# Cobalt-27/CompactFusion

Hardware: AMD Instinct MI355X
Metric: residual_compressed_activation_exchange_throughput (higher is better)
Workload: dtype f16

## Files before the change

compactfusion_amd/csrc/cfx_absmean.hip:

```cpp
#include <hip/hip_runtime.h>
#include <hip/hip_ext.h>
#include <stdint.h>
#include <stdio.h>
#include <stdlib.h>
#include <string.h>
#include <algorithm>
#include "cfx.h"
#include "cfx_internal.h"
#include "cfx_device.h"
#include "cfx_host.h"

#define CFX_I_FLAG_LR_FACTORS_ONLY 0x100
#define CFX_I_FLAG_LR_ABS 0x200
extern "C" CFX_HIDDEN size_t cfx_i_lr_workspace_bytes_any(int N, int C, int rank, int batch);
extern "C" CFX_HIDDEN void cfx_i_lr_factor_offsets(int N, int C, int rank, size_t* offU16, size_t* offV16, size_t* per);

template <bool EMIT_BITS, int US, bool WT = false, int NW = WAVES, bool PUB = false, bool KEEP = false, bool TAG = false, class E = ElemF16>
__device__ __forceinline__ void absmean_stats_body(const cfx_comp_item& it, int N, int C, int R, int CB, int bx, int by,
                                                   u64* rowpart, u64 (*sm)[TILE_C], Probe probe = Probe(),
                                                   h16x8* xk = nullptr, h16x8* bk = nullptr, TagArena ta = TagArena()) {
#define SSTAMP(k) probe.at(k)
    const TileCoord t = tile_coord_at(bx, by, N, C, R);
    const int cb = bx;
    u64* colpart = rowpart + (size_t)N * CB;
// ... 259 lines not shown
            const int r = t.r0 + t.w + j * WAVES;
            if (r >= t.r1) continue;
            h16 u[8];
#pragma unroll
            for (int k = 0; k < 8; ++k) u[k] = (k0 + k < K) ? U[(size_t)r * K + k0 + k] : (h16)0;
#pragma unroll
            for (int e = 0; e < 8; ++e)
#pragma unroll
                for (int k = 0; k < 8; ++k) acc[j][e] += (float)(h16)(u[k] * v[e][k]);
        }
    }
#pragma unroll
    for (int j = 0; j < RPT; ++j) {
        const int r = t.r0 + t.w + j * WAVES;
        if (r >= t.r1) continue;
        h16x8 bv = (h16x8)(h16)0, xv = (h16x8)(h16)0;
        if (base) bv = ld8(base + (size_t)r * C + t.c);
        unsigned byte;
        if (QUANT) {
            xv = ld8(x + (size_t)r * C + t.c);
            const h16x8 d = xv - bv;
            byte = 0;
#pragma unroll
            for (int i = 0; i < 8; ++i) byte |= (d[i] >= (h16)0 ? 1u : 0u) << i;
            pk[(size_t)r * C8 + (t.c >> 3)] = (unsigned char)byte;
        } else byte = pk[(size_t)r * C8 + (t.c >> 3)];
        if (!upd) continue;
        h16x8 o;
#pragma unroll
        for (int e = 0; e < 8; ++e) {
            const h16 sc = (h16)acc[j][e];
            const h16 recv = ((byte >> e) & 1u) ? sc : -sc;
            o[e] = base ? (h16)(bv[e] + recv) : recv;
        }
        if (QUANT && !ef) o = xv;
        st8(out + (size_t)r * C + t.c, o);
    }
}

#ifndef WATCH_SLEEP
#define WATCH_SLEEP 4
#endif
#ifndef INT2_FLAG_SLEEP
#define INT2_FLAG_SLEEP 2
#endif
__device__ __forceinline__ void scales_watch(const TagArena& ta, int N, int C, int c0, int r0, long long timeout) {
    const int tid = threadIdx.x;
    if (tid < 2) {
        const u64* w = tid ? ta.tU + min(r0, N - 1) : ta.tV + min(c0 + ((r0 >> 1) & (TILE_C - 1)), C - 1);
        SpinClock clk;
        while (!tag_is(ld_wt(w), ta.tagbits)) {
            __builtin_amdgcn_s_sleep(WATCH_SLEEP);
            if (clk.expired(timeout)) break;
        }
    }
    lds_barrier();
}
template <int ROWS, bool WATCH = true>
__device__ __forceinline__ bool scales_from_tagged(const TagArena& ta, int N, int C, int c0, int r0, u16* s16, long long timeout, unsigned* err) {
    static_assert(ROWS <= TILE_C, "one token word per thread (512 threads = the column block's channels)");
    const int tid = threadIdx.x;
    const u64* pv = ta.tV + min(c0 + tid, C - 1);
    const u64* pu = ta.tU + min(r0 + tid, N - 1);
    SpinClock clk;
    if (WATCH) scales_watch(ta, N, C, c0, r0, timeout);
    for (;;) {
        const u64 v = ld_wt(pv);
        const u64 u = tid < ROWS ? ld_wt(pu) : ta.tagbits;
        const bool ok = tag_is(v, ta.tagbits) && tag_is(u, ta.tagbits);
        s16[tid] = (u16)v;
        if (tid < ROWS) s16[TILE_C + tid] = (u16)u;
        if (!__syncthreads_or(ok ? 0 : 1)) return true;
        __builtin_amdgcn_s_sleep(2);
        if (__syncthreads_or(!ok && clk.expired(timeout) ? 1 : 0)) {
            if (tid == 0) gate_fail(err);
            return false;
        }
    }
}

#ifndef ONEBIT_D_TAGGED
#define ONEBIT_D_TAGGED 0
#endif
template <int NW, int KR, int KL, bool ST, class E = ElemF16>
__device__ __forceinline__ void binary_dequant_gated_body(const cfx_decomp_item& it, int N, int C, int R, int tile_x, int tile_y,
                                                         unsigned* gate, unsigned expect, unsigned* err, long long timeout, u32x4* lds,
                                                         Probe probe = Probe(), bool remote = false, bool tagged = false, TagArena ta = TagArena(),
                                                         u16* s16 = nullptr) {
    constexpr int K = KR + KL;
#define GSTAMP(k) do { if (ST && probe.on()) { asm volatile("s_waitcnt vmcnt(0)" ::: "memory"); probe.at(k); } } while (0)
    const TileCoord t = tile_coord_at(tile_x, tile_y, N, C, R);
    if (ST) { probe.at(0); probe.set(7, 4); }
    const unsigned char* pk = (const unsigned char*)it.packet;
    const int C8 = C >> 3;
    const u16* U = (const u16*)(pk + (size_t)N * C8);
    const u16* V = U + N;
    const h16* base = (const h16*)it.base;
    h16* out = (h16*)it.recon;
    const int cc = min(t.c, C - 8);
    h16x8 bv[KR];
    if (base) {
#pragma unroll
        for (int j = 0; j < KR; ++j) bv[j] = ld8nt(base + (size_t)min(t.r0 + t.w + NW * j, t.r1 - 1) * C + cc);
        if constexpr (KL > 0) {
            h16x8 tl[KL > 0 ? KL : 1];
#pragma unroll
            for (int j = 0; j < KL; ++j) tl[j] = ld8nt(base + (size_t)min(t.r0 + t.w + NW * (KR + j), t.r1 - 1) * C + cc);
#pragma unroll
            for (int j = 0; j < KL; ++j) lds[j * (NW * 64) + threadIdx.x] = __builtin_bit_cast(u32x4, tl[j]);
        }
    } else {
#pragma unroll
        for (int j = 0; j < KR; ++j) bv[j] = (h16x8)(h16)0;
    }
    GSTAMP(1);
    h16x8 v8;
    u16 ul;
    unsigned by[K];
    if (tagged) {
        scales_watch(ta, N, C, tile_x * TILE_C, t.r0, timeout);
        if (ST) probe.at(2);
#pragma unroll
        for (int j = 0; j < K; ++j) by[j] = ld_wt(pk + (size_t)min(t.r0 + t.w + NW * j, t.r1 - 1) * C8 + (cc >> 3));
        if (!scales_from_tagged<NW * K, false>(ta, N, C, tile_x * TILE_C, t.r0, s16, timeout, err)) return;
        v8 = __builtin_bit_cast(h16x8, *(const u16x8*)(s16 + 8 * t.lane));
        ul = s16[TILE_C + min(t.w + NW * min(t.lane, K - 1), t.r1 - 1 - t.r0)];
    } else if (!gate_wait<true>(gate, expect, err, timeout)) return;
    else if (remote) {
        if (ST) probe.at(2);
        u16x8 vb;
#pragma unroll
        for (int i = 0; i < 8; ++i) vb[i] = ld_sys(V + cc + i);
        v8 = __builtin_bit_cast(h16x8, vb);
        ul = ld_sys(U + min(t.r0 + t.w + NW * min(t.lane, K - 1), t.r1 - 1));
#pragma unroll
        for (int j = 0; j < K; ++j) by[j] = ld_sys(pk + (size_t)min(t.r0 + t.w + NW * j, t.r1 - 1) * C8 + (cc >> 3));
    } else {
        if (ST) probe.at(2);
        v8 = ld8_wt(V + cc);
        ul = ld_wt(U + min(t.r0 + t.w + NW * min(t.lane, K - 1), t.r1 - 1));
#pragma unroll
        for (int j = 0; j < K; ++j) by[j] = ld_wt(pk + (size_t)min(t.r0 + t.w + NW * j, t.r1 - 1) * C8 + (cc >> 3));
    }
    GSTAMP(3);
#pragma unroll
    for (int j = 0; j < K; ++j) {
        const int rr = t.r0 + t.w + NW * j;
        const h16 uj = hfrom((u16)__builtin_amdgcn_readlane((int)ul, j));
        if (rr < t.r1 && t.act) {
            const h16x8 s = v8 * uj;
            u16x8 sb = __builtin_bit_cast(u16x8, s);
#pragma unroll
            for (int i = 0; i < 8; ++i) sb[i] ^= ((by[j] >> i) & 1u) ? (u16)0 : (u16)0x8000;
            const h16x8 recv = __builtin_bit_cast(h16x8, sb);
            h16x8 bj = (h16x8)(h16)0;
            if (j < KR) bj = bv[j < KR ? j : 0];
            else if (base) bj = __builtin_bit_cast(h16x8, lds[(j - KR) * (NW * 64) + threadIdx.x]);
            st8nt(out + (size_t)rr * C + t.c, el_state<E>(base != nullptr, bj, recv));
        }
    }
    GSTAMP(4);
#undef GSTAMP
}

__device__ __forceinline__ void row_sums2_wt(const u64* rowpart, const unsigned* row32, int N, int CB, int m0, int m1, bool two, u64& s0, u64& s1) {
    s0 = 0; s1 = 0;
    for (int k0 = 0; k0 < CB; k0 += FUSED_RCH) {
        unsigned a[FUSED_RCH], b[FUSED_RCH];
#pragma unroll
        for (int j = 0; j < FUSED_RCH; ++j) a[j] = ld_wt(&row32[(size_t)min(k0 + j, CB - 1) * N + m0]);
        if (two) {
#pragma unroll
            for (int j = 0; j < FUSED_RCH; ++j) b[j] = ld_wt(&row32[(size_t)min(k0 + j, CB - 1) * N + m1]);
        } else {
#pragma unroll
            for (int j = 0; j < FUSED_RCH; ++j) b[j] = 0;
        }
        bool sat = false;
#pragma unroll
        for (int j = 0; j < FUSED_RCH; ++j) {
            s0 += (k0 + j < CB) ? a[j] : 0; s1 += (k0 + j < CB) ? b[j] : 0;
            sat |= (a[j] == PART_SAT) | (b[j] == PART_SAT);
        }
        if (sat) {
            for (int j = 0; j < FUSED_RCH && k0 + j < CB; ++j) {
                if (a[j] == PART_SAT) s0 += ld_wt(&rowpart[(size_t)(k0 + j) * N + m0]) - (u64)PART_SAT;
                if (two && b[j] == PART_SAT) s1 += ld_wt(&rowpart[(size_t)(k0 + j) * N + m1]) - (u64)PART_SAT;
            }
        }
    }
}

// ... 19 lines not shown
    }
    u64 keep0 = 0, keep1 = 0;
    if (last_all) row_sums2_wt(rowpart, row32, N, CB, min(tid, N - 1), min(tid + NT, N - 1), (tid & ~63) + NT < N, keep0, keep1);
    asm volatile("" ::: "memory");
    STAMP(4);
    u64* smem = &sm[1][0];
    float m0 = 0.f, m1 = 0.f;
    if (last_all) {
        const h16 h0 = mean16(keep0, C), h1 = mean16(keep1, C);
        m0 = (float)h0; m1 = (float)h1;
        u64 acc = 0;
        if (tid < N) acc += habs_units(hbits(h0));
        if (tid + NT < N) acc += habs_units(hbits(h1));
        for (int n0 = tid + 2 * NT; n0 - tid < N; n0 += 2 * NT) {
            const int n1 = n0 + NT;
            u64 s0, s1;
            row_sums2_wt(rowpart, row32, N, CB, min(n0, N - 1), min(n1, N - 1), (n1 & ~63) < N, s0, s1);
            if (n0 < N) acc += habs_units(hbits(mean16(s0, C)));
            if (n1 < N) acc += habs_units(hbits(mean16(s1, C)));
        }
        STAMP(13);
        u64 wtot;
        if (N <= 2 * NT) {
            const unsigned lo = wave_sum_u32_dpp((unsigned)(acc & 0xffffffu));
            const unsigned hi = wave_sum_u32_dpp((unsigned)(acc >> 24));
            wtot = ((u64)hi << 24) + lo;
        } else wtot = wave_sum_u64(acc);
        STAMP(14);
        if ((tid & 63) == 0) smem[tid >> 6] = wtot;
    }
    h16 vmean = (h16)0;
    if (last_col) {
        u64 a = 0;
        for (int p0 = 0; p0 < P; p0 += FUSED_CH) {
            if (p0) {
#pragma unroll
                for (int j = 0; j < FUSED_CH; ++j) v[j] = ld_wt(&col32[(size_t)min(p0 + j, P - 1) * C + cc]);
            }
            bool sat = false;
#pragma unroll
            for (int j = 0; j < FUSED_CH; ++j) { a += (p0 + j < P) ? v[j] : 0; sat |= v[j] == PART_SAT; }
            if (sat) {
                for (int j = 0; j < FUSED_CH && p0 + j < P; ++j)
                    if (v[j] == PART_SAT) a += ld_wt(&colpart[(size_t)(p0 + j) * C + cc]) - (u64)PART_SAT;
            }
        }
        vmean = mean16(a, N);
    }
    STAMP(5);
    if (last_all) {
        lds_barrier();
        STAMP(15);
        u64 tot = 0;
#pragma unroll
        for (int w = 0; w < NT / 64; ++w) tot += smem[w];
        const h16 mu = mean16(tot, N);
        const float den = eps_mode ? (float)(h16)((float)mu + 1e-6f) : (float)mu;
#define PUT16(ptr, val) do { const h16 _v = (val); if (GATED) st_wt((u16*)(ptr), hbits(_v)); else *(ptr) = _v; } while (0)
        if (tid < N) PUT16(&U[tid], (h16)(m0 / den));
        if (tid + NT < N) PUT16(&U[tid + NT], (h16)(m1 / den));
        for (int n0 = tid + 2 * NT; n0 - tid < N; n0 += 2 * NT) {
            const int n1 = n0 + NT;
            u64 s0, s1;
            row_sums2_wt(rowpart, row32, N, CB, min(n0, N - 1), min(n1, N - 1), (n1 & ~63) < N, s0, s1);
            if (n0 < N) PUT16(&U[n0], (h16)((float)mean16(s0, C) / den));
            if (n1 < N) PUT16(&U[n1], (h16)((float)mean16(s1, C) / den));
        }
        if (tid == 0) st_wt(tick + TICK_ALL, 0u);
    }
    if (last_col) {
        if (c < C) PUT16(&V[c], vmean);
        if (tid == 0) st_wt(tick + 1 + bx, 0u);
    }
#undef PUT16
    if (GATED) {
        asm volatile("s_waitcnt vmcnt(0)" ::: "memory");
        lds_barrier();
        if (tid == 0) gate_arrive_few(gate, (last_all ? 1u : 0u) + (last_col ? 1u : 0u));
    }
    STAMP(6);
#undef STAMP
}

__device__ __forceinline__ void absmean_tagged_jobs(const cfx_comp_item& it, int N, int C, int CB, int P, int bx, u64* rowpart, const TagArena& ta,
                                                    int per_byte, int eps_mode, u64 (*sm)[TILE_C], bool do_col, bool do_row, Probe probe,
                                                    unsigned* gate, unsigned* err, long long timeout) {
    constexpr int NT = FUSED_NT;
#define STAMP(k) probe.at(k)
    lds_barrier();
    const int tid = threadIdx.x;
    const u64* colpart = rowpart + (size_t)N * CB;
    h16* U = (h16*)((char*)it.packet + (size_t)N * (C / per_byte));
    h16* V = U + N;
    SpinClock clk;
    bool failed = false;
#define PUT16(ptr, val) st_wt((u16*)(ptr), hbits(val))
    if (do_col) {
        const int c = bx * TILE_C + tid, cc = min(c, C - 1);
        u64 a = 0;
        for (int p0 = 0; p0 < P && !failed; p0 += FUSED_CH) {
            u64 v[FUSED_CH];
            for (;;) {
#pragma unroll
                for (int j = 0; j < FUSED_CH; ++j) v[j] = ld_wt(&ta.tcol[(size_t)min(p0 + j, P - 1) * C + cc]);
                bool ok = true;
#pragma unroll
                for (int j = 0; j < FUSED_CH; ++j) ok = ok && tag_is(v[j], ta.tagbits);
                if (ok) break;
                __builtin_amdgcn_s_sleep(2);
                if (clk.expired(timeout)) { failed = true; break; }
            }
#pragma unroll
            for (int j = 0; j < FUSED_CH; ++j) {
                const u64 w = v[j] & TAG_SAT;
                if (p0 + j < P) a += (w == TAG_SAT && !failed) ? ld_wt(&colpart[(size_t)(p0 + j) * C + cc]) : w;
            }
        }
        STAMP(4);
        failed = __syncthreads_or(failed ? 1 : 0) != 0;
        if (!failed) {
            if (c < C) {
                const h16 vm = mean16(a, N);
                st_wt(&ta.tV[c], ta.tagbits | (u64)hbits(vm));
                PUT16(&V[c], vm);
            }
            asm volatile("s_waitcnt vmcnt(0)" ::: "memory");
            lds_barrier();
            if (tid == 0) gate_arrive_few(gate, 1u);
        }
        STAMP(5);
    }
    if (do_row && !failed) {
        u64* smem = &sm[1][0];
        auto row_sum = [&](int n) {
            const int nc = min(n, N - 1);
            u64 s_ = 0;
            for (int k0 = 0; k0 < CB && !failed; k0 += FUSED_RCH) {
                u64 q[FUSED_RCH];
                for (;;) {
#pragma unroll
                    for (int j = 0; j < FUSED_RCH; ++j) q[j] = ld_wt(&ta.trow[(size_t)min(k0 + j, CB - 1) * N + nc]);
                    bool ok = true;
#pragma unroll
                    for (int j = 0; j < FUSED_RCH; ++j) ok = ok && tag_is(q[j], ta.tagbits);
                    if (ok) break;
                    __builtin_amdgcn_s_sleep(2);
                    if (clk.expired(timeout)) { failed = true; break; }
                }
#pragma unroll
                for (int j = 0; j < FUSED_RCH; ++j) {
                    const u64 w = q[j] & TAG_SAT;
                    if (k0 + j < CB) s_ += (w == TAG_SAT && !failed) ? ld_wt(&rowpart[(size_t)(k0 + j) * N + nc]) : w;
                }
            }
            return s_;
        };
        h16 h0 = (h16)0, h1 = (h16)0;
        u64 acc = 0;
        for (int n0 = tid, i = 0; n0 - tid < N; n0 += NT, ++i) {
            const h16 h = mean16(row_sum(n0), C);
            if (i == 0) h0 = h;
            if (i == 1) h1 = h;
            if (n0 < N) acc += habs_units(hbits(h));
        }
        STAMP(13);
        const u64 wtot = wave_sum_u64(acc);
        if ((tid & 63) == 0) smem[tid >> 6] = wtot;
        failed = __syncthreads_or(failed ? 1 : 0) != 0;
        STAMP(15);
        if (!failed) {
            u64 tot = 0;
#pragma unroll
            for (int w = 0; w < NT / 64; ++w) tot += smem[w];
            const h16 mu = mean16(tot, N);
            const float den = eps_mode ? (float)(h16)((float)mu + 1e-6f) : (float)mu;
            for (int n0 = tid, i = 0; n0 < N; n0 += NT, ++i) {
                const h16 h = i == 0 ? h0 : (i == 1 ? h1 : mean16(row_sum(n0), C));
                const h16 un = (h16)((float)h / den);
                st_wt(&ta.tU[n0], ta.tagbits | (u64)hbits(un));
                PUT16(&U[n0], un);
            }
            asm volatile("s_waitcnt vmcnt(0)" ::: "memory");
            lds_barrier();
            if (tid == 0) gate_arrive_few(gate, 1u);
        }
        STAMP(6);
    }
#undef PUT16
#undef STAMP
    if (failed && tid == 0) gate_fail(err);
}

template <int US, class E = ElemF16>
__device__ __forceinline__ void own_tile_finish(const cfx_comp_item& it, int N, int C, int R, int bx, int by, int flags, const h16x8* xk,
                                                const h16x8* bk, unsigned* gate1, unsigned expect1, unsigned* gate2, unsigned expect2,
                                                unsigned* err, long long timeout, unsigned char* smw, const TagArena& ta, u16* s16) {
    constexpr int NW = FUSED_NW;
    static_assert(US * 8 <= 64, "a wave publishes its US rows of codes with 8 lanes a row");
    const TileCoord t = tile_coord_at(bx, by, N, C, R);
    h16* nb = (h16*)it.new_base;
    const bool upd = (flags & CFX_FLAG_UPDATE_CACHE) && nb;
    const bool ef = !(flags & CFX_FLAG_NO_EF);
    unsigned char* pk = (unsigned char*)it.packet;
    (void)gate1; (void)expect1;
    if (!scales_from_tagged<NW * US>(ta, N, C, bx * TILE_C, t.r0, s16, timeout, err)) return;
    const h16x8 ch8 = __builtin_bit_cast(h16x8, *(const u16x8*)(s16 + 8 * t.lane));
    const u16 ul = s16[TILE_C + min(t.w + NW * min(t.lane, US - 1), t.r1 - 1 - t.r0)];
    const bool has_base = it.base != nullptr;
    u16 codes[US];
#pragma unroll
    for (int j = 0; j < US; ++j) {
        const int rr = t.r0 + t.w + NW * j;
        const h16 tk = hfrom((u16)__builtin_amdgcn_readlane((int)ul, j));
        codes[j] = 0;
        if (rr < t.r1 && t.act) {
            const h16x8 d = el_diff<E>(xk[j], bk[j]);
            const h16x8 thr = ch8 * tk;
            const h16x8 a = habs8(d);
            unsigned code = 0;
#pragma unroll
            for (int i = 0; i < 8; ++i) {
                const unsigned sg = d[i] >= (h16)0 ? 1u : 0u;
                const unsigned m = a[i] > thr[i] ? 1u : 0u;
                code |= ((sg << 1) | m) << (2 * i);
            }
            codes[j] = (u16)code;
            ((u16*)smw)[j * 64 + t.lane] = (u16)code;
        }
    }
    {
        const int j = t.lane >> 3, seg = t.lane & 7;
        const int rr = t.r0 + t.w + NW * j;
        if (t.lane < 8 * US && rr < t.r1 && bx * TILE_C + seg * 64 < C)
            st16_wt(pk + (size_t)rr * (C >> 2) + bx * (TILE_C >> 2) + seg * 16, *(const u32x4*)(smw + j * 128 + seg * 16));
    }
    asm volatile("s_waitcnt vmcnt(0)" ::: "memory");
    lds_barrier();
    if (threadIdx.x == 0) {
        st_wt(&ta.tdone[(size_t)bx * ((N + R - 1) / R) + by], ta.tagbits);
        gate_arrive(gate2, 1u, expect2);
    }
    if (upd) {
#pragma unroll
        for (int j = 0; j < US; ++j) {
            const int rr = t.r0 + t.w + NW * j;
            const h16 tk = hfrom((u16)__builtin_amdgcn_readlane((int)ul, j));
            if (rr < t.r1 && t.act) {
                const h16x8 recv = int2_recv(codes[j], ch8 * tk);
                st8nt(nb + (size_t)rr * C + t.c, ef ? (el_state<E>(has_base, bk[j], recv)) : xk[j]);
            }
        }
    }
}

template <bool EMIT_BITS, int US, bool GATED = false, bool KEEP = false, class E = ElemF16>
__device__ __forceinline__ void absmean_fused_body(const cfx_comp_item& it, int N, int C, int R, int CB, int P, int bx, int by,
                                                   u64* rowpart, unsigned* tick, int per_byte, int eps_mode, u64 (*sm)[TILE_C], int dbg,
                                                   Probe probe, unsigned* gate = nullptr, unsigned gate_expect = 0, int flags = 0,
                                                   unsigned* gate2 = nullptr, unsigned expect2 = 0, unsigned* err = nullptr, long long timeout = 0,
                                                   TagArena ta = TagArena()) {
#define STAMP(k) probe.at(k)
    STAMP(0);
#ifdef CFX_DEV_PROBES
    if (dbg == 3) return;
    if (dbg == 4) {
        const TileCoord t = tile_coord_at(bx, by, N, C, R);
        h16x8 acc = (h16x8)(h16)0;
        for (int r = t.r0 + t.w; r < t.r1; r += FUSED_NW * US) {
            h16x8 xv[US], bv[US];
#pragma unroll
            for (int j = 0; j < US; ++j) {
                const int rr = min(r + FUSED_NW * j, t.r1 - 1);
                xv[j] = ld8nt((const h16*)it.x + (size_t)rr * C + min(t.c, C - 8));
                bv[j] = ld8((const h16*)it.base + (size_t)rr * C + min(t.c, C - 8));
            }
#pragma unroll
            for (int j = 0; j < US; ++j) acc += xv[j] - bv[j];
        }
        if (acc[0] == (h16)12345.0f) ((h16*)it.packet)[threadIdx.x] = acc[1];
        return;
    }
#endif
    h16x8 xk[KEEP ? US : 1], bk[KEEP ? US : 1];
    absmean_stats_body<EMIT_BITS, US, true, FUSED_NW, GATED, KEEP, GATED, E>(it, N, C, R, CB, bx, by, rowpart, sm, probe, xk, bk, ta);
    STAMP(1);
    if constexpr (GATED) {
        const bool v_wg = by == P - 1;
        const bool u_wg = P >= 2 ? (by == P - 2 && bx == CB - 1) : (bx == CB - 1);
        probe.copy(2, 1); probe.copy(3, 1); probe.set(7, (v_wg ? 1 : 0) | (u_wg ? 2 : 0));
        if (v_wg || u_wg) {
            u32x4* park = (u32x4*)&sm[FUSED_NW][0];
            if constexpr (KEEP) {
                park[threadIdx.x] = __builtin_bit_cast(u32x4, xk[US - 1]);
                park[FUSED_NT + threadIdx.x] = __builtin_bit_cast(u32x4, bk[US - 1]);
            }
            absmean_tagged_jobs(it, N, C, CB, P, bx, rowpart, ta, per_byte, eps_mode, sm, v_wg, u_wg, probe, gate, err, timeout);
            if constexpr (KEEP) {
                xk[US - 1] = __builtin_bit_cast(h16x8, park[threadIdx.x]);
                bk[US - 1] = __builtin_bit_cast(h16x8, park[FUSED_NT + threadIdx.x]);
            }
        }
    } else {
    asm volatile("s_waitcnt vmcnt(0)" ::: "memory");
    __syncthreads();
    STAMP(2);
#ifdef CFX_DEV_PROBES
    if (dbg == 1) return;
#endif
    unsigned* flag = (unsigned*)&sm[0][0];
    if (threadIdx.x == 0) flag[0] = __hip_atomic_fetch_add(tick + 1 + bx, 1u, __ATOMIC_RELAXED, __HIP_MEMORY_SCOPE_AGENT);
    if (threadIdx.x == 64) (void)__hip_atomic_fetch_add(tick + TICK_ALL, 1u, __ATOMIC_RELAXED, __HIP_MEMORY_SCOPE_AGENT);
    lds_barrier();
    const bool last_col = flag[0] == (unsigned)(P - 1);
    const bool u_wg = bx == 0 && by == 0;
    STAMP(3);
    probe.set(7, (last_col ? 1 : 0) | (u_wg ? 2 : 0));
#ifdef CFX_DEV_PROBES
    if (dbg == 2) {
        if (last_col && threadIdx.x == 0) st_wt(tick + 1 + bx, 0u);
        if (u_wg && threadIdx.x == 0) {
            while (ld_wt(tick + TICK_ALL) != (unsigned)(CB * P)) __builtin_amdgcn_s_sleep(1);
            st_wt(tick + TICK_ALL, 0u);
        }
        return;
    }
#endif
    if (last_col)
        absmean_last_arriver_jobs<GATED>(it, N, C, CB, P, bx, rowpart, tick, per_byte, eps_mode, sm, true, false, probe, gate, gate_expect);
    if (u_wg) {
        bool failed = false;
        if (threadIdx.x == 0) {
            SpinClock clk;
            while (ld_wt(tick + TICK_ALL) != (unsigned)(CB * P)) {
                __builtin_amdgcn_s_sleep(1);
                if (clk.expired(timeout)) { failed = true; gate_fail(err); break; }
            }
        }
        if (__syncthreads_or(failed ? 1 : 0)) return;
        absmean_last_arriver_jobs<GATED>(it, N, C, CB, P, bx, rowpart, tick, per_byte, eps_mode, sm, false, true, probe, gate, gate_expect);
    }
    }
    if constexpr (KEEP)
        own_tile_finish<US, E>(it, N, C, R, bx, by, flags, xk, bk, gate, gate_expect, gate2, expect2, err, timeout,
                                       (unsigned char*)&sm[__builtin_amdgcn_readfirstlane(threadIdx.x >> 6)][0], ta, (u16*)&sm[FUSED_NW + 4][0]);
#undef STAMP
}

struct FusedArgs {
    int N, C, CB, R, P;
    int n_st;
    int dq_R, dq_rb;
    int per_byte, eps_mode;
    int dbg;
    u64* ws;
    size_t ws_stride;
    unsigned* tick;
    Probe probe;
    int n_g, g_R, g_rb, n_gt;
    unsigned* gate;
    unsigned gate_expect;
    unsigned* gate_err;
    long long timeout;
    u64* tarena; size_t tarena_stride; unsigned tag;
    signed char src[CFX_MAX_BATCH];
    unsigned* xgate;
    unsigned xexpect;
    int remote;
    P2PInline p2p;
};
#ifndef GATE_WPE
#define GATE_WPE 4
#endif
template <bool EMIT_BITS, int US, bool GATED, bool ST, class E>
__global__ __launch_bounds__(FUSED_NT, GATE_WPE) __attribute__((amdgpu_num_vgpr(52))) void k_absmean_compress(BatchC batch, BatchD ride, BatchD gated, FusedArgs a) {
    __shared__ u64 sm[FUSED_NW][TILE_C];
    int b = blockIdx.x;
    if (b < a.n_st) {
        const int per = a.CB * a.P;
        const int z = b / per, rem = b - z * per;
        const int by = rem / a.CB;
        absmean_fused_body<EMIT_BITS, US, GATED, false, E>(batch.it[z], a.N, a.C, a.R, a.CB, a.P, rem - by * a.CB, by, a.ws + (size_t)z * a.ws_stride,
                                                 a.tick + z * TICK_WORDS, a.per_byte, a.eps_mode, sm, a.dbg,
                                                 a.probe.of(b), a.gate, a.gate_expect, 0, nullptr, 0u, a.gate_err, a.timeout,
                                                 tag_arena_of(a.tarena, a.tarena_stride, z, a.N, a.C, a.CB, a.P, a.tag));
        if constexpr (GATED) {
            if (b == 0 && a.p2p.own) p2p_exchange_inline(a.gate, a.gate_expect, 1, a.p2p, a.xgate, a.xexpect, a.gate_err);
        }
        return;
    }
    if constexpr (EMIT_BITS) {
        b -= a.n_st;
        if constexpr (GATED) {
            if (b < a.n_g) {
                const int per = a.CB * a.g_rb;
                for (int t = b; t < a.n_gt; t += a.n_g) {
                    const int item = t / per, rem = t - item * per;
                    const int ty = rem / a.CB;
                    const int sz = a.src[item];
                    const TagArena ta = tag_arena_of(a.tarena, a.tarena_stride, sz >= 0 ? sz : 0, a.N, a.C, a.CB, a.P, a.tag);
                    binary_dequant_gated_body<FUSED_NW, GATE_KR, 0, ST, E>(gated.it[item], a.N, a.C, a.g_R, rem - ty * a.CB, ty, a.xgate ? a.xgate : a.gate,
                                                                a.xgate ? a.xexpect : a.gate_expect, a.gate_err, a.timeout,
                                                                nullptr,
                                                                a.probe.of(blockIdx.x), a.remote != 0 && sz < 0,
                                                                ONEBIT_D_TAGGED && sz >= 0, ta, (u16*)&sm[0][0]);
                }
                return;
            }
            b -= a.n_g;
        }
        const int per = a.CB * a.dq_rb;
        const int item = b / per, rem = b - item * per;
        const int ty = rem / a.CB;
        binary_dequant_body<FUSED_NW, UNROLL, E>(ride.it[item], a.N, a.C, a.dq_R, rem - ty * a.CB, ty);
    }
}

#ifndef PIPE_US
#define PIPE_US 2
#endif
#define PIPE_MAX_DQ CFX_PIPE_MAX_DQ
struct BatchDX { cfx_decomp_item it[PIPE_MAX_DQ]; };
struct PipeArgs {
    int N, C, CB;
    int n_fin, fin_bpi, fin_P;
    int n_st, st_R, st_P;
    int dq_R, dq_rb;
    const u64* ws_fin;
    u64* ws_st;
    size_t ws_stride;
};
template <bool STEADY>
__global__ __launch_bounds__(NTHR) __attribute__((amdgpu_waves_per_eu(8, 8))) void k_binary_pipe(BatchDX dq, BatchC fin, BatchC st, PipeArgs a) {
    __shared__ u64 sm[WAVES][TILE_C];
    int b = blockIdx.x;
    if (b < a.n_fin) {
        const int item = b / a.fin_bpi;
        absmean_finalize_body<NTHR>(fin.it[item], a.N, a.C, a.CB, a.fin_P, 8, 0, a.ws_fin + (size_t)item * a.ws_stride, b - item * a.fin_bpi, &sm[0][0]);
        return;
    }
    b -= a.n_fin;
    if (b < a.n_st) {
        const int per = a.CB * a.st_P;
        const int item = b / per, rem = b - item * per;
        const int ty = rem / a.CB;
        absmean_stats_body<true, PIPE_US>(st.it[item], a.N, a.C, a.st_R, a.CB, rem - ty * a.CB, ty, a.ws_st + (size_t)item * a.ws_stride, sm);
        return;
    }
    b -= a.n_st;
    const int per = a.CB * a.dq_rb;
    const int item = b / per, rem = b - item * per;
    const int ty = rem / a.CB;
    binary_dequant_body<WAVES>(dq.it[item], a.N, a.C, a.dq_R, rem - ty * a.CB, ty);
}


template <class E>
__global__ __launch_bounds__(NTHR) void k_int2_quant(BatchC batch, int N, int C, int R, int flags) {
    const cfx_comp_item it = batch.it[blockIdx.z];
    const TileCoord t = tile_coord(N, C, R);
    const int C4 = C >> 2;
    unsigned char* pk = (unsigned char*)it.packet;
    const h16* TOK = (const h16*)(pk + (size_t)N * C4);
    const h16* CH = TOK + N;
    const h16* x = (const h16*)it.x;
    const h16* base = (const h16*)it.base;
    h16* nb = (h16*)it.new_base;
    const bool upd = (flags & CFX_FLAG_UPDATE_CACHE) && nb;
    const bool ef = !(flags & CFX_FLAG_NO_EF);
    const bool al16 = (((uintptr_t)CH) & 15) == 0;
    h16x8 ch8 = (h16x8)(h16)0;
    if (t.act) ch8 = ld8_tail(CH + t.c, al16);

    for (int r = t.r0 + t.w; r < t.r1; r += WAVES * UNROLL) {
        h16x8 xv[UNROLL], bv[UNROLL];
        h16 tk[UNROLL];
#pragma unroll
        for (int j = 0; j < UNROLL; ++j) {
            const int rr = r + WAVES * j;
            xv[j] = (h16x8)(h16)0; bv[j] = (h16x8)(h16)0; tk[j] = (h16)0;
            if (rr < t.r1 && t.act) {
                xv[j] = ld8nt(x + (size_t)rr * C + t.c);
                if (base) bv[j] = ld8nt(base + (size_t)rr * C + t.c);
                tk[j] = TOK[rr];
            }
        }
#pragma unroll
        for (int j = 0; j < UNROLL; ++j) {
            const int rr = r + WAVES * j;
            if (rr < t.r1 && t.act) {
                const h16x8 d = el_diff<E>(xv[j], bv[j]);
                const h16x8 thr = ch8 * tk[j];
                const h16x8 a = habs8(d);
                unsigned code = 0;
#pragma unroll
                for (int i = 0; i < 8; ++i) {
                    const unsigned s = d[i] >= (h16)0 ? 1u : 0u;
                    const unsigned m = a[i] > thr[i] ? 1u : 0u;
// ... 287 lines not shown
        Int2LayerArgs a;
        memset(&a, 0, sizeof(a));
        a.N = N; a.C = C; a.CB = CB; a.R = R; a.P = P; a.n_st = CB * P * batch;
        a.g_rb = (N + FUSED_NW * (GATE_KR2 + GATE_KL) - 1) / (FUSED_NW * (GATE_KR2 + GATE_KL));
        a.g_R = ((N + a.g_rb - 1) / a.g_rb + FUSED_NW - 1) / FUSED_NW * FUSED_NW;
        a.n_g = CB * a.g_rb * n_gated;
        a.flags = flags; a.ws = ws; a.ws_stride = wstride; a.tick = tick;
        a.gate1 = ctx->gate + (size_t)slot * GATE_STRIDE;
        a.gate2 = a.gate1 + GATE_BLOCK;
        ctx->gate_expect[3 * slot] += (unsigned)batch * (unsigned)(CB + 1);
        ctx->gate_expect[3 * slot + 1] += (unsigned)a.n_st;
        a.expect1 = ctx->gate_expect[3 * slot]; a.expect2 = ctx->gate_expect[3 * slot + 1];
        a.err = ctx->gate_err;
        a.timeout = ctx->gate_timeout;
        a.tarena_stride = tag_arena_words(N, C, CB, P);
        a.tag = abs_arena_for(ctx, slot / TICK_RING, stream, a.tarena_stride * batch * sizeof(u64), &a.tarena);
        if (!a.tag) return fail(ctx, CFX_ERR_LAUNCH, "2-bit layer launch: cannot allocate the partials' arena");
        for (int g_ = 0; g_ < n_gated; ++g_) {
            a.src[g_] = -1;
            for (int i = 0; i < batch; ++i)
                if (gd.it[g_].packet == items[i].packet) a.src[g_] = (signed char)i;
        }
        if (xg) {
            a.xgate = a.gate1 + 2 * GATE_BLOCK;
            a.xexpect = ++ctx->gate_expect[3 * slot + 2];
            a.remote = xg->remote;
            fill_p2p(ctx, xg, a.p2p);
            xg->taken = 1;
            xg->p_gate = a.gate2 + 1 * GATE_LINE;
            xg->p_expect = a.expect2;
            xg->f_gate = a.xgate; xg->f_expect = a.xexpect;
        }
        const dim3 g(a.n_st + a.n_g);
        LAUNCH_EL(bf16, ctx, KID_ABSMEAN_COMPRESS_GATED, s, (k_int2_compress_gated<4, EL>), g, dim3(FUSED_NT), 0, s, b, gd, a);
        return check_launch(ctx, "2-bit layer launch");
    }
    const bool ef_gated = one_launch && codec == CFX_CODEC_BINARY && upd && !(flags & CFX_FLAG_NO_EF) && n_gated + batch <= CFX_MAX_BATCH;
    const bool one_launch_1bit = one_launch && codec == CFX_CODEC_BINARY && (!upd || ef_gated);
    int n_gated_k = n_gated;
    if (ef_gated) {
        for (int i = n_gated - 1; i >= 0; --i) gd.it[i + batch] = gd.it[i];
        for (int i = 0; i < batch; ++i) { gd.it[i].packet = items[i].packet; gd.it[i].base = items[i].base; gd.it[i].recon = items[i].new_base; }
        n_gated_k = n_gated + batch;
    }
    if (fused) {
        FusedArgs a;
        memset(&a, 0, sizeof(a));
        a.N = N; a.C = C; a.CB = CB; a.R = R; a.P = P;
        a.n_st = CB * P * batch;
        a.dq_R = FUSED_NW * UNROLL;
        a.dq_rb = (N + a.dq_R - 1) / a.dq_R;
        a.per_byte = per_byte; a.eps_mode = codec == CFX_CODEC_INT2 ? 1 : 0;
        a.ws = ws; a.ws_stride = wstride; a.tick = tick;
        a.dbg = ctx->dev_probe;
        a.probe = cfx_i_probe(ctx);
        if (one_launch_1bit) {
            a.g_rb = (N + FUSED_NW * GATE_KR - 1) / (FUSED_NW * GATE_KR);
            a.g_R = ((N + a.g_rb - 1) / a.g_rb + FUSED_NW - 1) / FUSED_NW * FUSED_NW;
            a.n_gt = a.n_g = CB * a.g_rb * n_gated_k;
            a.gate = ctx->gate + (size_t)slot * GATE_STRIDE;
            ctx->gate_expect[3 * slot] += (unsigned)batch * (unsigned)(CB + 1);
            a.gate_expect = ctx->gate_expect[3 * slot];
            a.tarena_stride = tag_arena_words(N, C, CB, P);
            a.tag = abs_arena_for(ctx, slot / TICK_RING, stream, a.tarena_stride * batch * sizeof(u64), &a.tarena);
            if (!a.tag) return fail(ctx, CFX_ERR_LAUNCH, "1-bit layer launch: cannot allocate the partials' arena");
            for (int g_ = 0; g_ < n_gated_k; ++g_) {
                a.src[g_] = -1;
                for (int i = 0; i < batch; ++i)
                    if (gd.it[g_].packet == items[i].packet) a.src[g_] = (signed char)i;
            }
            if (xg) {
                a.xgate = a.gate + GATE_BLOCK;
                a.xexpect = ++ctx->gate_expect[3 * slot + 1];
                a.remote = xg->remote;
                fill_p2p(ctx, xg, a.p2p);
                xg->taken = 1;
                xg->p_gate = a.gate; xg->p_expect = a.gate_expect;
                xg->f_gate = a.xgate; xg->f_expect = a.xexpect;
            }
        }
        a.gate_err = ctx->gate_err;
        a.timeout = ctx->gate_timeout;
        const dim3 g(a.n_st + a.n_g + CB * a.dq_rb * n_ride);
#ifdef CFX_DEV_PROBES
        if (one_launch_1bit && ctx->dev_buf && R % 32 == 0) {
            LAUNCH_EL(bf16, ctx, KID_ABSMEAN_COMPRESS_GATED, s, (k_absmean_compress<true, 4, true, true, EL>), g, dim3(FUSED_NT), 0, s, b, rd, gd, a);
        } else
#endif
        if (one_launch_1bit) {
            LAUNCH_EL(bf16, ctx, KID_ABSMEAN_COMPRESS_GATED, s, (k_absmean_compress<true, 4, true, false, EL>), g, dim3(FUSED_NT), 0, s, b, rd, gd, a);
        } else if (codec == CFX_CODEC_BINARY) {
            if (R % 32 == 0) LAUNCH_EL(bf16, ctx, KID_ABSMEAN_COMPRESS_BITS, s, (k_absmean_compress<true, 4, false, false, EL>), g, dim3(FUSED_NT), 0, s, b, rd, gd, a);
            else LAUNCH_EL(bf16, ctx, KID_ABSMEAN_COMPRESS_BITS, s, (k_absmean_compress<true, 2, false, false, EL>), g, dim3(FUSED_NT), 0, s, b, rd, gd, a);
        } else {
            if (R % 32 == 0) LAUNCH_EL(bf16, ctx, KID_ABSMEAN_COMPRESS, s, (k_absmean_compress<false, 4, false, false, EL>), g, dim3(FUSED_NT), 0, s, b, rd, gd, a);
            else LAUNCH_EL(bf16, ctx, KID_ABSMEAN_COMPRESS, s, (k_absmean_compress<false, 2, false, false, EL>), g, dim3(FUSED_NT), 0, s, b, rd, gd, a);
        }
    } else {
        if (codec == CFX_CODEC_BINARY) LAUNCH_EL(bf16, ctx, KID_ABSMEAN_STATS_BITS, s, (k_absmean_stats<true, EL>), grid, dim3(NTHR), 0, s, b, N, C, R, ws, wstride);
        else LAUNCH_EL(bf16, ctx, KID_ABSMEAN_STATS, s, (k_absmean_stats<false, EL>), grid, dim3(NTHR), 0, s, b, N, C, R, ws, wstride);
        LAUNCH(ctx, KID_ABSMEAN_FINALIZE, s, k_absmean_finalize, dim3(1 + (C + 255) / 256, batch), dim3(1024), 0, s, b, N, C, CB, P, per_byte,
                           codec == CFX_CODEC_INT2 ? 1 : 0, (const u64*)ws, wstride);
        if (n_ride) {
            const int Rr = auto_rows(ctx, N, C, n_ride, false);
            LAUNCH_EL(bf16, ctx, KID_BINARY_DEQUANT, s, (k_binary_dequant<UNROLL, EL>), dim3(CB, (N + Rr - 1) / Rr, n_ride), dim3(NTHR), 0, s, rd, N, C, Rr, (unsigned*)nullptr, 0u);
        }
    }
    if (codec == CFX_CODEC_INT2) {
        LAUNCH_EL(bf16, ctx, KID_INT2_QUANT, s, (k_int2_quant<EL>), gridq, dim3(NTHR), 0, s, b, N, C, Rq, flags);
    } else if (upd && !one_launch_1bit) {
        if (flags & CFX_FLAG_NO_EF) {
            for (int i = 0; i < batch; ++i)
                if (items[i].new_base != items[i].x)
                    hipLaunchKernelGGL(k_copy_probe, dim3(2048), dim3(256), 0, s, (uint4*)items[i].new_base, (const uint4*)items[i].x, (size_t)N * C * 2 / 16);
        } else {
            BatchD d;
            memset(&d, 0, sizeof(d));
            for (int i = 0; i < batch; ++i) { d.it[i].packet = items[i].packet; d.it[i].base = items[i].base; d.it[i].recon = items[i].new_base; }
            LAUNCH_EL(bf16, ctx, KID_BINARY_EF, s, (k_binary_dequant<UNROLL, EL>), gridq, dim3(NTHR), 0, s, d, N, C, Rq, (unsigned*)nullptr, 0u);
        }
    }
    if (n_gated && !(one_launch_1bit || (one_launch && codec == CFX_CODEC_INT2))) {
        const int Rg = auto_rows(ctx, N, C, n_gated, false);
        if (codec == CFX_CODEC_BINARY) LAUNCH_EL(bf16, ctx, KID_BINARY_DEQUANT, s, (k_binary_dequant<UNROLL, EL>), dim3(CB, (N + Rg - 1) / Rg, n_gated), dim3(NTHR), 0, s, gd, N, C, Rg, (unsigned*)nullptr, 0u);
        else LAUNCH_EL(bf16, ctx, KID_INT2_DEQUANT, s, (k_int2_dequant<EL>), dim3(CB, (N + Rg - 1) / Rg, n_gated), dim3(NTHR), 0, s, gd, N, C, Rg, (unsigned*)nullptr, 0u);
    }
    return check_launch(ctx, "compress launch");
}

int cfx_i_absmean_decompress(cfx_ctx* ctx, int codec, bool bf16, int N, int C, int batch, const BatchD& b, int R, void* stream, unsigned* pre, unsigned pre_val) {
    hipStream_t s = (hipStream_t)stream;
    const dim3 grid((C + TILE_C - 1) / TILE_C, (N + R - 1) / R, batch);
    if (codec == CFX_CODEC_BINARY) {
        if (stream_cu_count(ctx, stream) < 128) {
            const int R4 = WAVES * 4;
            LAUNCH_EL(bf16, ctx, KID_BINARY_DEQUANT, s, (k_binary_dequant<4, EL>), dim3(grid.x, (N + R4 - 1) / R4, batch), dim3(NTHR), 0, s, b, N, C, R4, pre, pre_val);
        } else LAUNCH_EL(bf16, ctx, KID_BINARY_DEQUANT, s, (k_binary_dequant<UNROLL, EL>), grid, dim3(NTHR), 0, s, b, N, C, R, pre, pre_val);
    } else LAUNCH_EL(bf16, ctx, KID_INT2_DEQUANT, s, (k_int2_dequant<EL>), grid, dim3(NTHR), 0, s, b, N, C, R, pre, pre_val);
    return check_launch(ctx, "decompress launch");
}

extern "C" {

int cfx_int2_quantize(cfx_ctx* ctx, int N, int C, int flags, int batch, const cfx_comp_item* items, void* stream) {
    const bool bf16 = (flags & CFX_FLAG_ELEM_BF16) != 0;
    if (!ctx || !items) return fail(ctx, CFX_ERR_NULL, "int2_quantize: null ctx/items");
    if (batch < 1 || batch > CFX_MAX_BATCH) return fail(ctx, CFX_ERR_BATCH, "int2_quantize: batch out of range");
    if (!shape_ok(CFX_CODEC_INT2, N, C, 0)) return fail(ctx, CFX_ERR_SHAPE, "int2_quantize: bad shape");
    const bool upd = flags & CFX_FLAG_UPDATE_CACHE;
    BatchC b;
    memset(&b, 0, sizeof(b));
    for (int i = 0; i < batch; ++i) {
        if (!items[i].x || !items[i].packet) return fail(ctx, CFX_ERR_NULL, "int2_quantize: null x/packet");
        if (upd && !items[i].new_base) return fail(ctx, CFX_ERR_NULL, "int2_quantize: UPDATE_CACHE needs new_base");
        if (!AL16(items[i].x) || !AL16(items[i].base) || !AL16(items[i].new_base) || !AL16(items[i].packet))
            return fail(ctx, CFX_ERR_ALIGN, "int2_quantize: pointers must be 16-byte aligned");
        b.it[i] = items[i];
    }
    hipStream_t s = (hipStream_t)stream;
    const int Rq = auto_rows(ctx, N, C, batch, true);
    LAUNCH_EL(bf16, ctx, KID_INT2_QUANT, s, (k_int2_quant<EL>), dim3((C + TILE_C - 1) / TILE_C, (N + Rq - 1) / Rq, batch), dim3(NTHR), 0, s, b, N, C, Rq, flags);
    return check_launch(ctx, "int2 quantise launch");
}
}

int cfx_i_launch_pipe(cfx_plan* p, hipStream_t s, int N, int C, const int* comp_op, const int* deq_op,
                       const PipeUnit* dq, const PipeUnit* fin, const PipeUnit* st, int fin_parity, int st_parity,
                       hipEvent_t done_ev) {
    cfx_ctx* ctx = p->ctx;
    BatchDX bd; BatchC bf, bs;
    PipeArgs a;
    memset(&a, 0, sizeof(a));
// ... 118 lines not shown
```

compactfusion_amd/csrc/cfx_device.h:

```cpp
#ifndef CFX_DEVICE_H
#define CFX_DEVICE_H
#include <hip/hip_runtime.h>
#include <stdint.h>
#include "cfx.h"
#include "cfx_internal.h"

typedef _Float16 h16;
typedef h16 h16x8 __attribute__((ext_vector_type(8)));
typedef unsigned short u16;
typedef u16 u16x8 __attribute__((ext_vector_type(8)));
typedef unsigned long long u64;
typedef unsigned u32x4 __attribute__((ext_vector_type(4)));
typedef float f32x2 __attribute__((ext_vector_type(2)));
typedef h16 h16x2 __attribute__((ext_vector_type(2)));
typedef __bf16 bf16x2 __attribute__((ext_vector_type(2)));

#define TILE_C 512
#define WAVES 4
#define NTHR (WAVES * 64)
#define UNROLL 2
#define UNROLL_S 4

struct BatchC { cfx_comp_item it[CFX_MAX_BATCH]; };
struct BatchD { cfx_decomp_item it[CFX_MAX_BATCH]; };
// ... 153 lines not shown
        return __builtin_bit_cast(h16x8, o);
    }
}

template <class E>
__device__ __forceinline__ void el_widen8(h16x8 v, float (&f)[8]) {
    if constexpr (!E::bf16) {
#pragma unroll
        for (int k = 0; k < 8; ++k) f[k] = (float)v[k];
    } else {
        const u32x4 w = __builtin_bit_cast(u32x4, v);
#pragma unroll
        for (int i = 0; i < 4; ++i) {
            const f32x2 p = bf2_f32(w[i]);
            f[2 * i] = p[0];
            f[2 * i + 1] = p[1];
        }
    }
}
template <class E>
__device__ __forceinline__ h16x8 el_round8(const float (&f)[8]) {
    u32x4 o;
#pragma unroll
    for (int i = 0; i < 4; ++i) {
        const f32x2 p = {f[2 * i], f[2 * i + 1]};
        if constexpr (E::bf16) o[i] = f32_bf2(p);
        else o[i] = __builtin_bit_cast(unsigned, __builtin_convertvector(p, h16x2));
    }
    return __builtin_bit_cast(h16x8, o);
}

__device__ __forceinline__ h16x8 int2_recv(u16 code, h16x8 thr) {
    h16x8 r;
#pragma unroll
    for (int i = 0; i < 8; ++i) {
        const unsigned idx = (code >> (2 * i)) & 3u;
        const h16 lvl = (idx & 1u) ? (h16)2.0 * thr[i] : (h16)0.5 * thr[i];
        r[i] = (idx & 2u) ? lvl : -lvl;
    }
    return r;
}

struct TileCoord {
    int lane, w, c, r0, r1;
    bool act;
};
__device__ __forceinline__ TileCoord tile_coord_at(int bx, int by, int N, int C, int R) {
    TileCoord t;
    t.lane = threadIdx.x & 63;
    t.w = __builtin_amdgcn_readfirstlane(threadIdx.x >> 6);
    t.c = bx * TILE_C + t.lane * 8;
    t.act = t.c < C;
    t.r0 = by * R;
    t.r1 = min(N, t.r0 + R);
    return t;
}
__device__ __forceinline__ TileCoord tile_coord(int N, int C, int R) { return tile_coord_at(blockIdx.x, blockIdx.y, N, C, R); }

#define MML_MAX_TILES 2048
#define TICK_WORDS 64
#define TICK_ALL 48
#define TICK_MAX_CB 46
#define TICK_RING 256

#define FUSED_NW 8
#define FUSED_NT (FUSED_NW * 64)
#ifndef FUSED_CH
#define FUSED_CH 18

#endif
#define FUSED_RCH 6

#ifndef GATE_KR
#define GATE_KR 14
#endif
#ifndef GATE_KR2
#define GATE_KR2 17

#endif
#ifndef GATE_KL
#define GATE_KL 6
#endif
#define GATE_LDS_ROWS ((GATE_KL * FUSED_NT * 16 + TILE_C * 8 - 1) / (TILE_C * 8))
#ifndef GATE_LOCAL_SLEEP
#define GATE_LOCAL_SLEEP 1

#endif
#define GATE_LINE 16
#define GATE_BLOCK (25 * GATE_LINE)
#define GATE_STRIDE (3 * GATE_BLOCK)
__device__ __forceinline__ void gate_arrive_few(unsigned* gate, unsigned inc) {
    (void)__hip_atomic_fetch_add(gate, inc, __ATOMIC_RELAXED, __HIP_MEMORY_SCOPE_AGENT);
}
__device__ __forceinline__ void gate_arrive(unsigned* gate, unsigned inc, unsigned expect) {
    const unsigned old = __hip_atomic_fetch_add(gate, inc, __ATOMIC_RELAXED, __HIP_MEMORY_SCOPE_AGENT);
    if (old + inc == expect) {
#pragma unroll
        for (int x = 0; x < 8; ++x) st_wt(gate + (1 + x) * GATE_LINE, expect);
    }
}
__device__ __forceinline__ unsigned ld_l2(const unsigned* p) {
    unsigned v;
    asm volatile("global_load_dword %0, %1, off nt\n\ts_waitcnt vmcnt(0)" : "=&v"(v) : "v"(p) : "memory");
    return v;
}
struct SpinClock {
    long long t0 = 0;
    __device__ __forceinline__ bool expired(long long timeout) {
        const long long now = wall_clock64();
        if (!t0) { t0 = now; return false; }
        return now - t0 > timeout;
    }
};
template <bool FEW = false>
__device__ __forceinline__ bool gate_wait(unsigned* gate, unsigned expect, unsigned* err, long long timeout) {
    bool failed = false;
    if (threadIdx.x == 0) {
        const unsigned xcc = __builtin_amdgcn_s_getreg((3 << 11) | 20) & 7u;
        unsigned* open = FEW ? gate : gate + (1 + xcc) * GATE_LINE;
        unsigned* local = gate + (9 + xcc) * GATE_LINE;
        unsigned* claim = gate + (17 + xcc) * GATE_LINE;
        const bool relay = __hip_atomic_exchange(claim, expect, __ATOMIC_RELAXED, __HIP_MEMORY_SCOPE_AGENT) != expect;
        SpinClock clk;
        unsigned n = 0;
        if (relay) {
            while (ld_wt(open) != expect) {
                __builtin_amdgcn_s_sleep(1);
                if (clk.expired(timeout)) { failed = true; break; }
            }
            if (!failed) *(volatile unsigned*)local = expect;
        } else {
            while (ld_l2(local) != expect) {
                if (GATE_LOCAL_SLEEP) __builtin_amdgcn_s_sleep(GATE_LOCAL_SLEEP);
                ++n;
                if ((n & (FEW ? 255u : 15u)) == 0) {
                    if (ld_wt(open) == expect) break;
                    if (clk.expired(timeout)) { failed = true; break; }
                }
            }
        }
        if (failed) gate_fail(err);
    }
    return __syncthreads_or(failed ? 1 : 0) == 0;
}
__device__ __forceinline__ h16x8 ld8_wt(const u16* p) {
    if ((((uintptr_t)p) & 7) == 0) {
        struct { u64 a, b; } q = {ld_wt((const u64*)p), ld_wt((const u64*)p + 1)};
        return __builtin_bit_cast(h16x8, q);
    }
    u16x8 vb;
#pragma unroll
    for (int i = 0; i < 8; ++i) vb[i] = ld_wt(p + i);
    return __builtin_bit_cast(h16x8, vb);
}

struct P2PInline {
    unsigned* own;
    const unsigned* peer[CFX_P2P_MAX_PEERS];
    int n_peers;
    long long timeout;
};
__device__ __forceinline__ unsigned ld_sys32(const unsigned* p) { return __hip_atomic_load(p, __ATOMIC_RELAXED, __HIP_MEMORY_SCOPE_SYSTEM); }
__device__ __forceinline__ void p2p_exchange_inline(const unsigned* p_gate, unsigned p_expect, int p_count, const P2PInline& p,
                                                    unsigned* f_gate, unsigned f_expect, unsigned* err) {
    if ((threadIdx.x >> 6) != 0) return;
    const int lane = threadIdx.x & 63;
// ... 44 lines not shown
```

Before: 2117.

## Add dense gated compress kernel parking base rows in LDS with staged loads

Adds a k_absmean_compress_dense variant used when the grid fits within a per-CU budget. It keeps fewer base rows in registers (40 VGPRs, higher waves per EU) and parks the remaining rows in shared memory, with each gated block handling exactly one tile instead of looping. It also loads the first rows, waits on them, and then issues the rest. A lean variant of the tagged column wait precomputes a byte offset to cut address arithmetic. The intent is higher occupancy and better latency hiding, at the cost of extra LDS traffic and a forced vmcnt wait.

```diff
diff --git a/compactfusion_amd/csrc/cfx_absmean.hip b/compactfusion_amd/csrc/cfx_absmean.hip
--- a/compactfusion_amd/csrc/cfx_absmean.hip
+++ b/compactfusion_amd/csrc/cfx_absmean.hip
@@ -365,7 +365,7 @@
 #ifndef ONEBIT_D_TAGGED
 #define ONEBIT_D_TAGGED 0
 #endif
-template <int NW, int KR, int KL, bool ST, class E = ElemF16>
+template <int NW, int KR, int KL, bool ST, class E = ElemF16, int STAGE = 0>
 __device__ __forceinline__ void binary_dequant_gated_body(const cfx_decomp_item& it, int N, int C, int R, int tile_x, int tile_y,
                                                          unsigned* gate, unsigned expect, unsigned* err, long long timeout, u32x4* lds,
                                                          Probe probe = Probe(), bool remote = false, bool tagged = false, TagArena ta = TagArena(),
@@ -373,7 +373,7 @@
     constexpr int K = KR + KL;
 #define GSTAMP(k) do { if (ST && probe.on()) { asm volatile("s_waitcnt vmcnt(0)" ::: "memory"); probe.at(k); } } while (0)
     const TileCoord t = tile_coord_at(tile_x, tile_y, N, C, R);
-    if (ST) { probe.at(0); probe.set(7, 4); }
+    if (ST) { probe.at(0); probe.set(7, 4); probe.set(8, (KL << 8) | STAGE); }
     const unsigned char* pk = (const unsigned char*)it.packet;
     const int C8 = C >> 3;
     const u16* U = (const u16*)(pk + (size_t)N * C8);
@@ -383,14 +383,28 @@
     const int cc = min(t.c, C - 8);
     h16x8 bv[KR];
     if (base) {
-#pragma unroll
-        for (int j = 0; j < KR; ++j) bv[j] = ld8nt(base + (size_t)min(t.r0 + t.w + NW * j, t.r1 - 1) * C + cc);
-        if constexpr (KL > 0) {
+        if constexpr (STAGE > 0) {
+            static_assert(STAGE <= KR, "the staged rows stay in registers");
+#pragma unroll
+            for (int j = 0; j < STAGE; ++j) bv[j] = ld8nt(base + (size_t)min(t.r0 + t.w + NW * j, t.r1 - 1) * C + cc);
+            asm volatile("s_waitcnt vmcnt(0)" ::: "memory");
             h16x8 tl[KL > 0 ? KL : 1];
 #pragma unroll
             for (int j = 0; j < KL; ++j) tl[j] = ld8nt(base + (size_t)min(t.r0 + t.w + NW * (KR + j), t.r1 - 1) * C + cc);
 #pragma unroll
+            for (int j = STAGE; j < KR; ++j) bv[j] = ld8nt(base + (size_t)min(t.r0 + t.w + NW * j, t.r1 - 1) * C + cc);
+#pragma unroll
             for (int j = 0; j < KL; ++j) lds[j * (NW * 64) + threadIdx.x] = __builtin_bit_cast(u32x4, tl[j]);
+        } else {
+#pragma unroll
+            for (int j = 0; j < KR; ++j) bv[j] = ld8nt(base + (size_t)min(t.r0 + t.w + NW * j, t.r1 - 1) * C + cc);
+            if constexpr (KL > 0) {
+                h16x8 tl[KL > 0 ? KL : 1];
+#pragma unroll
+                for (int j = 0; j < KL; ++j) tl[j] = ld8nt(base + (size_t)min(t.r0 + t.w + NW * (KR + j), t.r1 - 1) * C + cc);
+#pragma unroll
+                for (int j = 0; j < KL; ++j) lds[j * (NW * 64) + threadIdx.x] = __builtin_bit_cast(u32x4, tl[j]);
+            }
         }
     } else {
 #pragma unroll
@@ -576,6 +590,7 @@
 #undef STAMP
 }
 
+template <bool LEAN = false>
 __device__ __forceinline__ void absmean_tagged_jobs(const cfx_comp_item& it, int N, int C, int CB, int P, int bx, u64* rowpart, const TagArena& ta,
                                                     int per_byte, int eps_mode, u64 (*sm)[TILE_C], bool do_col, bool do_row, Probe probe,
                                                     unsigned* gate, unsigned* err, long long timeout) {
@@ -594,9 +609,13 @@
         u64 a = 0;
         for (int p0 = 0; p0 < P && !failed; p0 += FUSED_CH) {
             u64 v[FUSED_CH];
+            unsigned off = (unsigned)cc * 8u;
             for (;;) {
-#pragma unroll
-                for (int j = 0; j < FUSED_CH; ++j) v[j] = ld_wt(&ta.tcol[(size_t)min(p0 + j, P - 1) * C + cc]);
+                if (LEAN) asm volatile("" : "+v"(off));
+#pragma unroll
+                for (int j = 0; j < FUSED_CH; ++j)
+                    v[j] = LEAN ? ld_wt((const u64*)((const char*)(ta.tcol + (size_t)min(p0 + j, P - 1) * C) + off))
+                                : ld_wt(&ta.tcol[(size_t)min(p0 + j, P - 1) * C + cc]);
                 bool ok = true;
 #pragma unroll
                 for (int j = 0; j < FUSED_CH; ++j) ok = ok && tag_is(v[j], ta.tagbits);
@@ -747,7 +766,7 @@
     }
 }
 
-template <bool EMIT_BITS, int US, bool GATED = false, bool KEEP = false, class E = ElemF16>
+template <bool EMIT_BITS, int US, bool GATED = false, bool KEEP = false, class E = ElemF16, bool LEAN = false>
 __device__ __forceinline__ void absmean_fused_body(const cfx_comp_item& it, int N, int C, int R, int CB, int P, int bx, int by,
                                                    u64* rowpart, unsigned* tick, int per_byte, int eps_mode, u64 (*sm)[TILE_C], int dbg,
                                                    Probe probe, unsigned* gate = nullptr, unsigned gate_expect = 0, int flags = 0,
@@ -788,7 +807,7 @@
                 park[threadIdx.x] = __builtin_bit_cast(u32x4, xk[US - 1]);
                 park[FUSED_NT + threadIdx.x] = __builtin_bit_cast(u32x4, bk[US - 1]);
             }
-            absmean_tagged_jobs(it, N, C, CB, P, bx, rowpart, ta, per_byte, eps_mode, sm, v_wg, u_wg, probe, gate, err, timeout);
+            absmean_tagged_jobs<LEAN>(it, N, C, CB, P, bx, rowpart, ta, per_byte, eps_mode, sm, v_wg, u_wg, probe, gate, err, timeout);
             if constexpr (KEEP) {
                 xk[US - 1] = __builtin_bit_cast(h16x8, park[threadIdx.x]);
                 bk[US - 1] = __builtin_bit_cast(h16x8, park[FUSED_NT + threadIdx.x]);
@@ -865,15 +884,16 @@
 #ifndef GATE_WPE
 #define GATE_WPE 4
 #endif
-template <bool EMIT_BITS, int US, bool GATED, bool ST, class E>
-__global__ __launch_bounds__(FUSED_NT, GATE_WPE) __attribute__((amdgpu_num_vgpr(52))) void k_absmean_compress(BatchC batch, BatchD ride, BatchD gated, FusedArgs a) {
-    __shared__ u64 sm[FUSED_NW][TILE_C];
+template <bool EMIT_BITS, int US, bool GATED, bool ST, class E, int KR, int KL, int STAGE>
+__device__ __forceinline__ void absmean_compress_launch(const BatchC& batch, const BatchD& ride, const BatchD& gated, const FusedArgs& a,
+                                                        u64 (*sm)[TILE_C], u32x4* park) {
+    constexpr bool DENSE = KL > 0;
     int b = blockIdx.x;
     if (b < a.n_st) {
         const int per = a.CB * a.P;
         const int z = b / per, rem = b - z * per;
         const int by = rem / a.CB;
-        absmean_fused_body<EMIT_BITS, US, GATED, false, E>(batch.it[z], a.N, a.C, a.R, a.CB, a.P, rem - by * a.CB, by, a.ws + (size_t)z * a.ws_stride,
+        absmean_fused_body<EMIT_BITS, US, GATED, false, E, DENSE>(batch.it[z], a.N, a.C, a.R, a.CB, a.P, rem - by * a.CB, by, a.ws + (size_t)z * a.ws_stride,
                                                  a.tick + z * TICK_WORDS, a.per_byte, a.eps_mode, sm, a.dbg,
                                                  a.probe.of(b), a.gate, a.gate_expect, 0, nullptr, 0u, a.gate_err, a.timeout,
                                                  tag_arena_of(a.tarena, a.tarena_stride, z, a.N, a.C, a.CB, a.P, a.tag));
@@ -887,17 +907,19 @@
         if constexpr (GATED) {
             if (b < a.n_g) {
                 const int per = a.CB * a.g_rb;
-                for (int t = b; t < a.n_gt; t += a.n_g) {
+                auto tile = [&](int t) {
                     const int item = t / per, rem = t - item * per;
                     const int ty = rem / a.CB;
                     const int sz = a.src[item];
                     const TagArena ta = tag_arena_of(a.tarena, a.tarena_stride, sz >= 0 ? sz : 0, a.N, a.C, a.CB, a.P, a.tag);
-                    binary_dequant_gated_body<FUSED_NW, GATE_KR, 0, ST, E>(gated.it[item], a.N, a.C, a.g_R, rem - ty * a.CB, ty, a.xgate ? a.xgate : a.gate,
+                    binary_dequant_gated_body<FUSED_NW, KR, KL, ST, E, STAGE>(gated.it[item], a.N, a.C, a.g_R, rem - ty * a.CB, ty, a.xgate ? a.xgate : a.gate,
                                                                 a.xgate ? a.xexpect : a.gate_expect, a.gate_err, a.timeout,
-                                                                nullptr,
+                                                                park,
                                                                 a.probe.of(blockIdx.x), a.remote != 0 && sz < 0,
                                                                 ONEBIT_D_TAGGED && sz >= 0, ta, (u16*)&sm[0][0]);
-                }
+                };
+                if constexpr (DENSE) tile(b);
+                else for (int t = b; t < a.n_gt; t += a.n_g) tile(t);
                 return;
             }
             b -= a.n_g;
@@ -907,6 +929,18 @@
         const int ty = rem / a.CB;
         binary_dequant_body<FUSED_NW, UNROLL, E>(ride.it[item], a.N, a.C, a.dq_R, rem - ty * a.CB, ty);
     }
+}
+template <bool EMIT_BITS, int US, bool GATED, bool ST, class E>
+__global__ __launch_bounds__(FUSED_NT, GATE_WPE) __attribute__((amdgpu_num_vgpr(52))) void k_absmean_compress(BatchC batch, BatchD ride, BatchD gated, FusedArgs a) {
+    __shared__ u64 sm[FUSED_NW][TILE_C];
+    absmean_compress_launch<EMIT_BITS, US, GATED, ST, E, GATE_KR, 0, GATE_STAGE == 2 ? GATE_STAGE_ROWS : 0>(batch, ride, gated, a, sm, nullptr);
+}
+template <bool ST, class E>
+__global__ __launch_bounds__(FUSED_NT, GATE_DENSE_WPE) __attribute__((amdgpu_num_vgpr(40))) void k_absmean_compress_dense(BatchC batch, BatchD ride, BatchD gated, FusedArgs a) {
+    static_assert(!ONEBIT_D_TAGGED, "the tagged scales' LDS words would alias the parked rows");
+    static_assert(GATE_DENSE_KL >= 0 && GATE_DENSE_KR >= GATE_STAGE_ROWS, "GATE_DENSE_KR rows in registers, the others of GATE_KR parked");
+    __shared__ u64 sm[GATE_DENSE_LDS_ROWS > FUSED_NW ? GATE_DENSE_LDS_ROWS : FUSED_NW][TILE_C];
+    absmean_compress_launch<true, 4, true, ST, E, GATE_DENSE_KR, GATE_DENSE_KL, GATE_STAGE ? GATE_STAGE_ROWS : 0>(batch, ride, gated, a, sm, (u32x4*)&sm[0][0]);
 }
 
 #ifndef PIPE_US
@@ -1360,12 +1394,17 @@
         a.gate_err = ctx->gate_err;
         a.timeout = ctx->gate_timeout;
         const dim3 g(a.n_st + a.n_g + CB * a.dq_rb * n_ride);
+        const bool dense = GATE_DENSE && one_launch_1bit && R % 32 == 0 && !(xg && xg->needs_room) &&
+                           (long)g.x <= (long)GATE_DENSE_PER_CU * stream_cus;
 #ifdef CFX_DEV_PROBES
         if (one_launch_1bit && ctx->dev_buf && R % 32 == 0) {
-            LAUNCH_EL(bf16, ctx, KID_ABSMEAN_COMPRESS_GATED, s, (k_absmean_compress<true, 4, true, true, EL>), g, dim3(FUSED_NT), 0, s, b, rd, gd, a);
+            if (dense) LAUNCH_EL(bf16, ctx, KID_ABSMEAN_COMPRESS_GATED, s, (k_absmean_compress_dense<true, EL>), g, dim3(FUSED_NT), 0, s, b, rd, gd, a);
+            else LAUNCH_EL(bf16, ctx, KID_ABSMEAN_COMPRESS_GATED, s, (k_absmean_compress<true, 4, true, true, EL>), g, dim3(FUSED_NT), 0, s, b, rd, gd, a);
         } else
 #endif
-        if (one_launch_1bit) {
+        if (dense) {
+            LAUNCH_EL(bf16, ctx, KID_ABSMEAN_COMPRESS_GATED, s, (k_absmean_compress_dense<false, EL>), g, dim3(FUSED_NT), 0, s, b, rd, gd, a);
+        } else if (one_launch_1bit) {
             LAUNCH_EL(bf16, ctx, KID_ABSMEAN_COMPRESS_GATED, s, (k_absmean_compress<true, 4, true, false, EL>), g, dim3(FUSED_NT), 0, s, b, rd, gd, a);
         } else if (codec == CFX_CODEC_BINARY) {
             if (R % 32 == 0) LAUNCH_EL(bf16, ctx, KID_ABSMEAN_COMPRESS_BITS, s, (k_absmean_compress<true, 4, false, false, EL>), g, dim3(FUSED_NT), 0, s, b, rd, gd, a);
diff --git a/compactfusion_amd/csrc/cfx_device.h b/compactfusion_amd/csrc/cfx_device.h
--- a/compactfusion_amd/csrc/cfx_device.h
+++ b/compactfusion_amd/csrc/cfx_device.h
@@ -259,6 +259,20 @@
 #define GATE_KL 6
 #endif
 #define GATE_LDS_ROWS ((GATE_KL * FUSED_NT * 16 + TILE_C * 8 - 1) / (TILE_C * 8))
+#ifndef GATE_DENSE
+#define GATE_DENSE 1
+#endif
+#ifndef GATE_DENSE_KR
+#define GATE_DENSE_KR 10
+#endif
+#define GATE_DENSE_KL (GATE_KR - GATE_DENSE_KR)
+#define GATE_DENSE_WPE 6
+#define GATE_DENSE_PER_CU 3
+#define GATE_DENSE_LDS_ROWS ((GATE_DENSE_KL * FUSED_NT * 16 + TILE_C * 8 - 1) / (TILE_C * 8))
+#ifndef GATE_STAGE
+#define GATE_STAGE 1
+#endif
+#define GATE_STAGE_ROWS 2
 #ifndef GATE_LOCAL_SLEEP
 #define GATE_LOCAL_SLEEP 1
 
```

After: 1993. 0.942x the previous value.
